# flanglet/kanzi-cpp

Hardware: AMD Instinct MI355X
Metric: encode+decode MB/s on the synthetic stand-in for silesia.tar (bit-exact) (higher is better)
Workload: dtype u8

## Files before the change

kanzi-cpp_amd/csrc/bwt_fwd.hip:

```cpp
#include "common.hpp"
#include "stages.hpp"
#include "bwt_common.hpp"

#include <cstdlib>
#include <cstring>
#include <algorithm>
#include <cmath>
#include "prims.hpp"
#include <chrono>
#include <vector>

namespace knz {

constexpr u32 SM_TS = 1792;
constexpr u32 SM_WIN = 2048;
constexpr u32 SM_G = 256;
constexpr u32 MED_CAP = 8192;
constexpr u32 MED_LO_CAP = 2048;
constexpr u32 SUPER_CAP = 8192;
constexpr int GATHER_THREADS = 512;
constexpr u32 GATHER_ROWS = 16;
static_assert(MED_CAP <= GATHER_ROWS * GATHER_THREADS, "k_bwt_f_gather_desc judges a medium group from one batch of loads");
constexpr u32 LARGE_OS_MIN = 1000000;
constexpr u32 NO_BIT = 0x7FFFFFFFu;
// ... 440 lines not shown
            if (tid + o < 64) sm = u < sm ? u : sm;
        }
        int pex = __shfl_up(pm, 1, 64);
        if (tid == 0) pex = -1;
        u32 sex = (u32)__shfl_down((int)sm, 1, 64);
        if (tid == 63) sex = NO_BIT;
        W.prevSet[tid] = pex;
        W.nextSet[tid] = sex;
        const bool zero = (tid < (int)(SM_TS / 32)) ? (w != 0xFFFFFFFFu) : (tid == (int)(SM_TS / 32) ? ((w & 1u) == 0) : false);
        const unsigned long long anyz = __ballot(zero);
        if (tid == 0) *sAny = anyz != 0 ? 1 : 0;
    }
    __syncthreads();
    return *sAny != 0;
}

__device__ __forceinline__ bool sm_group_of(const SmWindow& W, u32 i, u32& s, u32& e)
{
    const u32 w = i >> 5, bit = i & 31;
    const u32 lowmask = (bit == 31) ? 0xFFFFFFFFu : ((2u << bit) - 1u);
    const u32 word = W.bw[w];
    const u32 m = word & lowmask;
    int si = m ? (int)(w * 32 + 31 - __clz((int)m)) : W.prevSet[w];
    if (si < 0 || (u32)si >= SM_TS) return false;
    const u32 m2 = word & ~lowmask;
    const u32 ei = m2 ? (w * 32 + (u32)__ffs((int)m2) - 1) : W.nextSet[w];
    if (ei == NO_BIT) return false;
    const u32 len = ei - (u32)si;
    if (len < 2 || len > SM_G) return false;
    s = (u32)si; e = ei;
    return true;
}

__global__ __launch_bounds__(256) void k_bwt_f_r0_place_text(BwtView bv, FwdView v, const u32* __restrict__ winLastIncl, const u32* __restrict__ winFirstInclRev, u32 nWin,
                                                             uint2* __restrict__ largeNext, const u64* __restrict__ keys, int nsym, int pbits, uint2* __restrict__ runList,
                                                             const u32* __restrict__ gapTab)
{
    __shared__ SmWindow W;
    __shared__ int sBlk;
    __shared__ ClassAgg A;
    __shared__ u32 sSA[SM_WIN];
    __shared__ u64 sK[SM_WIN];
    __shared__ u32 sNew[64];
    __shared__ u32 sAfterLocal;
    constexpr int E = (int)(SM_WIN / 256);
    constexpr u32 TSW = SM_TS / 32;
    const int tid = (int)threadIdx.x;
    const u32 win = blockIdx.x;
    const u32 slot0 = win * SM_TS;
    if (tid == 0) sBlk = find_block(v.base, v.nBlocks, slot0 < v.total ? slot0 : v.total - 1);
    agg_init(A);
    if (tid < 64) {
        sNew[tid] = 0;
        const u32 w = v.gbits[(slot0 >> 5) + (u32)tid];
        W.bw[tid] = w;
        int pm = w ? (tid * 32 + 31 - __clz((int)w)) : -1;
        u32 sm = w ? (u32)(tid * 32 + __ffs((int)w) - 1) : NO_BIT;
        for (int o = 1; o < 64; o <<= 1) {
            const int t = __shfl_up(pm, (unsigned)o, 64);
            if (tid >= o) pm = t > pm ? t : pm;
            const u32 u = (u32)__shfl_down((int)sm, (unsigned)o, 64);
            if (tid + o < 64) sm = u < sm ? u : sm;
        }
        int pex = __shfl_up(pm, 1u, 64);
        if (tid == 0) pex = -1;
        u32 sex = (u32)__shfl_down((int)sm, 1u, 64);
        if (tid == 63) sex = NO_BIT;
        W.prevSet[tid] = pex;
        W.nextSet[tid] = sex;
    } else if (tid < 128) {
        const int k = tid - 64;
        const u32 w = (k < (int)(2 * TSW - 64)) ? v.gbits[(slot0 >> 5) + 64u + (u32)k] : 0u;
        const unsigned long long any = __ballot(w != 0);
        const int first = any ? __ffsll((long long)any) - 1 : 0;
        if (k == first) sAfterLocal = any ? SM_WIN + (u32)k * 32u + (u32)__ffs((int)w) - 1u : NO_BIT;
    }
    __syncthreads();
    const u32 before = win ? winLastIncl[win - 1] : 0u;
    u32 after = (sAfterLocal != NO_BIT) ? slot0 + sAfterLocal : ((win + 2 < nWin) ? winFirstInclRev[nWin - 3 - win] : v.total);
    if (after > v.total) after = v.total;
    const u64 pmask = (1ull << pbits) - 1ull;
    u32 gp[E], gs[E], ge[E];
    u64 kk[E];
    bool inView[E], mine[E];
    int blkOf[E];
#pragma unroll
    for (int k = 0; k < E; k++) {
        const u32 i = (u32)tid + 256u * (u32)k;
        const u32 a = slot0 + i;
        inView[k] = a < v.total;
        mine[k] = false; gp[k] = 0; kk[k] = 0; gs[k] = 0; ge[k] = 0; blkOf[k] = 0;
        if (!inView[k]) continue;
        int blk = sBlk;
        while (a >= v.base[blk + 1]) blk++;
        blkOf[k] = blk;
        kk[k] = keys[a];
        gp[k] = v.base[blk] + (u32)(kk[k] & pmask);
        mine[k] = sm_group_of(W, i, gs[k], ge[k]);
        if (mine[k]) {
            const u32 bb = v.base[blk], n = v.base[blk + 1] - bb;
            const u32 q = gp[k] - bb + (u32)nsym;
            const u8* t = bv.src[blk];
            const u64 x = text8(t, q, n);
            sSA[i] = gp[k];
            sK[i] = (__builtin_bswap64(x) & ~0xFFull) | (u64)(i - gs[k]);
        }
    }
    __syncthreads();
    u32 surv = 0;
    int hKind[E];
    u32 hLocal[E], hSize[E];
#pragma unroll
    for (int k = 0; k < E; k++) {
        const u32 i = (u32)tid + 256u * (u32)k;
        const u32 a = slot0 + i;
        hKind[k] = -1; hLocal[k] = 0; hSize[k] = 0;
        if (!inView[k]) continue;
        if (mine[k]) {
            const u64 ki = sK[i], lo = ki & ~0xFFull;
            u32 less = 0, rank = 0;
            for (u32 j = gs[k]; j < ge[k]; j++) {
                const u64 kj = sK[j];
                rank += (kj < ki) ? 1u : 0u;
                less += (kj < lo) ? 1u : 0u;
            }
            const u32 eqBefore = rank - less;
            const u32 headIdx = gs[k] + less;
            v.SA[slot0 + headIdx + eqBefore] = gp[k];
            lab_set(v, gp[k], v.base[blkOf[k]], slot0 + headIdx, slot0 + headIdx);
            if (less != 0 && eqBefore == 0) atomicOr(&sNew[headIdx >> 5], 1u << (headIdx & 31));
            if (eqBefore != 0) surv = 1;
            continue;
        }
        if (i >= SM_TS) continue;
        const u32 w = i >> 5, bit = i & 31;
        const u32 lowmask = (bit == 31) ? 0xFFFFFFFFu : ((2u << bit) - 1u);
        const u32 word = W.bw[w];
// ... 1784 lines not shown
        __syncthreads();
#pragma unroll
        for (u32 q = 0; q < RUN_ROWS / 4; q++) {
            const u32 row = wave + 4 * q;
            if (row >= nRows) break;
            const u32 Rend = rowMax[q] < c0 + RUN_CH - 1 ? rowMax[q] : c0 + RUN_CH - 1;
            for (u32 R = c0; R <= Rend; R++) {
                const bool alive = Lr[q] >= R;
                const unsigned long long m = __ballot(alive);
                const u32 j = segBase + colBase[R - c0] + cnt[row][R - c0] + (u32)__popcll(m & __lanemask_lt());
                if (alive && j < M) {
                    keys[j] = kb[q] | ((above ? hiAll - (u64)R : (u64)R) << kbits);
                    vals[j] = e[q] - R;
                    Rout[j] = R;
                }
            }
        }
        __syncthreads();
    }
}

__global__ __launch_bounds__(256) void k_bwt_f_run_flags(const u64* __restrict__ keys, u32 M, unsigned long long* __restrict__ bits64)
{
    const u32 j = blockIdx.x * 256 + threadIdx.x;
    const u64 k = (j < M) ? keys[j] : 0ull;
    u32 klo = (u32)__shfl_up((int)(u32)k, 1u, 64), khi = (u32)__shfl_up((int)(u32)(k >> 32), 1u, 64);
    u64 kp = ((u64)khi << 32) | klo;
    if ((threadIdx.x & 63) == 0 && j > 0 && j < M) kp = keys[j - 1];
    const bool f = (j >= M) || (j == 0) || (k != kp);
    const unsigned long long m = __ballot(f);
    if ((threadIdx.x & 63) == 0) bits64[j >> 6] = m;
}

__global__ __launch_bounds__(256) void k_bwt_f_run_place(FwdView v, const uint2* __restrict__ desc, const u32* __restrict__ loff, u32 M, int kbits, const u64* __restrict__ keys,
                                                         const u32* __restrict__ vals, const u32* __restrict__ bits, const u32* __restrict__ winLastIncl,
                                                         const u32* __restrict__ winFirstInclRev, u32 nWin, uint2* __restrict__ largeNext, const u32* __restrict__ memberR,
                                                         u32* __restrict__ ovr, u32* __restrict__ rtbits, const u32* __restrict__ lbase, int allLabels)
{
    __shared__ SmWindow W;
    __shared__ ClassAgg A;
    const int tid = (int)threadIdx.x;
    const u32 jb = blockIdx.x * 256u;
    const u32 win = jb / SM_WIN, j0 = win * SM_WIN;
    agg_init(A);
    if (tid < 64) {
        const u32 w = bits[(j0 >> 5) + (u32)tid];
        W.bw[tid] = w;
        int pm = w ? (tid * 32 + 31 - __clz((int)w)) : -1;
        u32 sm = w ? (u32)(tid * 32 + __ffs((int)w) - 1) : NO_BIT;
        for (int o = 1; o < 64; o <<= 1) {
            const int t = __shfl_up(pm, (unsigned)o, 64);
            if (tid >= o) pm = t > pm ? t : pm;
            const u32 u = (u32)__shfl_down((int)sm, (unsigned)o, 64);
            if (tid + o < 64) sm = u < sm ? u : sm;
        }
        int pex = __shfl_up(pm, 1u, 64);
        if (tid == 0) pex = -1;
        u32 sex = (u32)__shfl_down((int)sm, 1u, 64);
        if (tid == 63) sex = NO_BIT;
        W.prevSet[tid] = pex;
        W.nextSet[tid] = sex;
    }
    __syncthreads();
    const u32 j = jb + (u32)tid;
    u32 surv = 0, mySlot = 0, hLocal = 0, hSize = 0;
    int hKind = -1;
    bool setBit = false;
    if (j < M) {
        const u32 i = j - j0;
        const u32 w = i >> 5, bit = i & 31;
        const u32 lowmask = (bit == 31) ? 0xFFFFFFFFu : ((2u << bit) - 1u);
        const u32 word = W.bw[w];
        const u32 m = word & lowmask;
        const int si = m ? (int)(w * 32 + 31 - (u32)__clz((int)m)) : W.prevSet[w];
        const u32 nh = (si >= 0) ? j0 + (u32)si : (win ? winLastIncl[win - 1] : 0u);
        const u32 di = (u32)(keys[j] >> kbits);
        const u32 gs = desc[di].x, off = loff[di];
        const u32 gp = vals[j];
        mySlot = gs + (j - off);
        v.SA[mySlot] = gp;
        if (nh != off || allLabels) lab_set(v, gp, lbase[di], gs + (nh - off), gs);
        ovr[mySlot] = memberR[j];
        if (nh == j) {
            const u32 m2 = word & ~lowmask;
            const u32 ei = m2 ? (w * 32 + (u32)__ffs((int)m2) - 1) : W.nextSet[w];
            u32 nxt = (ei != NO_BIT) ? j0 + ei : ((win + 1 < nWin) ? winFirstInclRev[nWin - 2 - win] : M);
            if (nxt > M) nxt = M;
            setBit = (j != off);
            hSize = nxt - j;
            hKind = agg_note(A, hSize, false, surv, hLocal);
        }
    }
    if (__ballot(surv != 0) != 0 && (tid & 63) == 0) v.counters[CNT_SMALL_LEFT] = 1;
    __syncthreads();
    if (tid == 0) agg_reserve(A, v);
    __syncthreads();
    if (hKind >= 0) agg_write(A, v, hKind, hLocal, mySlot, hSize, largeNext, (uint2*)nullptr);
    const int lane = tid & 63;
    const bool live = j < M;
    const u32 s0 = (u32)__shfl((int)mySlot, 0, 64);
    const bool inLine = live && (mySlot == s0 + (u32)lane);
    const unsigned long long hm = __ballot(setBit && inLine), rm = __ballot(inLine);
    if (live && !inLine) {
        if (setBit) atomicOr(&v.gnew[mySlot >> 5], 1u << (mySlot & 31));
        atomicOr(&rtbits[mySlot >> 5], 1u << (mySlot & 31));
    }
    if (lane == 0) {
        const u32 w0 = s0 >> 5, sh = s0 & 31;
        for (int which = 0; which < 2; which++) {
            const unsigned long long mask = which ? rm : hm;
            u32* dst = which ? rtbits : v.gnew;
            if (mask == 0) continue;
            const u32 p0 = (u32)(mask << sh);
            const u32 p1 = sh ? (u32)(mask >> (32 - sh)) : (u32)(mask >> 32);
            const u32 p2 = sh ? (u32)(mask >> (64 - sh)) : 0u;
            if (p0) atomicOr(&dst[w0], p0);
            if (p1) atomicOr(&dst[w0 + 1], p1);
            if (p2) atomicOr(&dst[w0 + 2], p2);
        }
// ... 48 lines not shown
        d[0] = (u8)((logNbChunks << 2) | (pIndexSize - 1));
        u32 idx = 1;
        for (int k = 0; k < chunks; k++) {
            const u32 prim = lab_cur(fv, bb + (u32)k * step, bb) - bb;
            for (int sh = (int)(pIndexSize - 1) * 8; sh >= 0; sh -= 8) d[idx++] = (u8)(prim >> sh);
        }
        newLen[b] = hdr + n;
    }
}

__global__ __launch_bounds__(256) void k_bwt_f_med_flags(const uint2* __restrict__ stage, u32 nSlots, u32* __restrict__ flags)
{
    const u32 i = blockIdx.x * 256 + threadIdx.x;
    if (i >= nSlots) return;
    const u32 n = stage[i].y;
    flags[i] = (n != 0 && n <= MED_LO_CAP) ? 1u : 0u;
    flags[nSlots + i] = (n > MED_LO_CAP) ? 1u : 0u;
}

__global__ __launch_bounds__(256) void k_bwt_f_med_compact(uint2* __restrict__ stage, u32 nSlots, const u32* __restrict__ prefix, uint2* __restrict__ medNext,
                                                           u32 at, u32* __restrict__ idxLo, u32 atLo, u32* __restrict__ idxHi, u32 atHi, u32* __restrict__ nLoOut)
{
    const u32 i = blockIdx.x * 256 + threadIdx.x;
    if (i >= nSlots) return;
    const u32 nLo = prefix[nSlots];
    if (i == 0) *nLoOut = nLo;
    const uint2 d = stage[i];
    if (d.y == 0) return;
    const u32 pLo = prefix[i], pHi = prefix[nSlots + i] - nLo, g = at + pLo + pHi;
    medNext[g] = d; stage[i] = make_uint2(0u, 0u);
    if (d.y <= MED_LO_CAP) idxLo[atLo + pLo] = g; else idxHi[atHi + pHi] = g;
}

struct FwdTuning { int nsym; int noRunRound; int runFallback; int stats; int link; int plainLabels; int noPack; int noUnsplitSkip; int noGroupSleep; int noMediumFuse; int runSort; int chainList; int runInSort; };
static FwdTuning& fwd_tuning()
{
    static FwdTuning t = [] {
        FwdTuning x; x.nsym = 0; x.noRunRound = 0; x.runFallback = 0; x.stats = 0; x.link = 1; x.plainLabels = 0; x.noPack = 0; x.noUnsplitSkip = 0; x.noGroupSleep = 0; x.noMediumFuse = 0; x.runSort = 0; x.chainList = 0; x.runInSort = 0;
        if (getenv("KNZ_BWT_PLAIN_LABELS")) x.plainLabels = 1;
        if (getenv("KNZ_BWT_NO_PACK")) x.noPack = 1;
        if (getenv("KNZ_BWT_NO_UNSPLIT_SKIP")) x.noUnsplitSkip = 1;
        if (getenv("KNZ_BWT_NO_GROUP_SLEEP")) x.noGroupSleep = 1;
        if (getenv("KNZ_BWT_NO_MEDIUM_FUSE")) x.noMediumFuse = 1;
        if (const char* e = getenv("KNZ_BWT_RUN_SORT")) x.runSort = atoi(e);
        if (const char* e = getenv("KNZ_BWT_CHAIN_LIST")) x.chainList = atoi(e);
        if (const char* e = getenv("KNZ_BWT_RUN_IN_SORT")) x.runInSort = atoi(e);
        if (const char* e = getenv("KNZ_BWT_LINK")) x.link = atoi(e);
        if (getenv("KNZ_BWT_STATS")) x.stats = 1;
        if (const char* e = getenv("KNZ_BWT_NSYM")) x.nsym = atoi(e);
        if (getenv("KNZ_BWT_NO_RUN_ROUND")) x.noRunRound = 1;
        if (getenv("KNZ_BWT_RUN_FALLBACK")) x.runFallback = 1;
        return x;
    }();
    return t;
}
int bwt_forward_tune(const char* key, int value)
{
    FwdTuning& t = fwd_tuning();
    if (!strcmp(key, "rs_onesweep")) { prims::rs_onesweep_knob().store(value); return 0; }
    if (!strcmp(key, "bwt_nsym")) t.nsym = value;
    else if (!strcmp(key, "bwt_no_run_round")) t.noRunRound = value;
    else if (!strcmp(key, "bwt_run_fallback")) t.runFallback = value;
    else if (!strcmp(key, "bwt_stats")) t.stats = value;
    else if (!strcmp(key, "bwt_link")) t.link = value;
    else if (!strcmp(key, "bwt_plain_labels")) t.plainLabels = value;
    else if (!strcmp(key, "bwt_no_pack")) t.noPack = value;
    else if (!strcmp(key, "bwt_no_unsplit_skip")) t.noUnsplitSkip = value;
    else if (!strcmp(key, "bwt_no_group_sleep")) t.noGroupSleep = value;
    else if (!strcmp(key, "bwt_no_medium_fuse")) t.noMediumFuse = value;
    else if (!strcmp(key, "bwt_run_sort")) t.runSort = value;
    else if (!strcmp(key, "bwt_chain_list")) t.chainList = value;
    else if (!strcmp(key, "bwt_run_in_sort")) t.runInSort = value;
    else return -1;
    return 0;
}

struct FwdScratch {
    u64* keysA; u64* keysB;
    u32* valsA; u32* valsB;
    u32* SA; u32* ISA; u32* K; u64* ISA2;
    u32* t0; u32* t1; u32* t2; u32* t3;
    u32* gbits; u32* gnew; u32* rtbits; u32* ovr; size_t gbitsWords;
    uint2* med[2]; uint2* medStage; uint2* medVerdict[2]; u32* medFlags; u32* medPrefix; u32* medIdxLo; u32* medIdxHi; size_t medSlots; uint2* descInfo; uint2* large[2]; uint2* runList; uint4* superList; u32* ebits;
    u32* loff; u32* lbase;
    u32* survTile;
    u32* linkedTile;
    u32* base;
    u32* counters;
    u32* seg2;
    void* scanTmp;
    void* rsMem;
    u32* byteHist;
    u32* classTab; u32* rbits; u32* rcount; u32* rprefix;
    u32* runPos; u32* runE; u32* runL; u32* sE; u32* rcnt; u32* moff;
    u64* runKeysA; u64* runKeysB; u64* sKey;
    u32* runTileStart; u32* runColTab;
    u32* gapMembers; u32* gapFirst; u32* gapStart; u32* cbase;
    size_t maxRuns;
};

static size_t fwd_align(size_t x) { return (x + 255) & ~(size_t)255; }

static size_t fwd_carve(u8* p, int nBlocks, size_t total, FwdScratch* w, u32 VS)
{
    u8* q = p;
// ... 67 lines not shown
        if (mode == OFF && h >= retryH) mode = UNTRIED;
        if (mode == UNTRIED && survMembers >= total / 8) { mode = TRIAL; trials++; return true; }
        if (mode == ON && survMembers >= total / 64) { mode = APPLIED; return true; }
        return false;
    }
};

struct FwdSort {
    hipStream_t s; const XfStage& st; u32* hp;
    const FwdTuning tune = fwd_tuning();
    BwtView bv; FwdView v; FwdScratch w; size_t maxTotal;
    prims::RsWs rs1;
    u32 total, medSlots, nTiles; int nsym, pbits, kbits;
    bool groupSleep = false;
    u32 h = 1; int cur = 0;
    u64 *keysFree, *keysFree2;
    bool medFuse = false;
    bool runDirect = false;
    bool gaps = false;
    u32 gapClasses = 0, keptOut = 0, scanRuns = 0, scanLongest = 0;
    u32 nMedLo = 0;
    u32 nRun, runElems, surv, nMed, nLarge, largeElems, survMembers;
    LinkPlan link; LinkTrial linkTr; std::chrono::steady_clock::time_point statT;
    int fetch(u32 first, u32 n) { return hipMemcpyAsync(hp + first, w.counters + first, 4 * (size_t)n, hipMemcpyDeviceToHost, s) == hipSuccess && hipStreamSynchronize(s) == hipSuccess ? 0 : -1; }
    void merge_bits() { hipLaunchKernelGGL(k_bwt_f_merge_bits, GRID1(total / 32 + 2), w.gbits, w.gnew, total / 32 + 2); }
    void enable_run_tiebits() { if (!v.rtbits) { hipMemsetAsync(w.rtbits, 0, 4 * w.gbitsWords, s); v.ovr = w.ovr; v.rtbits = w.rtbits; } }
    void compact_medium(uint2* dst, u32 at = 0, u32 atLo = 0)
    {
        KScope ks_("k_bwt_f_med_compact");
        hipLaunchKernelGGL(k_bwt_f_med_flags, GRID1(medSlots), w.medStage, medSlots, w.medFlags);
        prims::launch_scan<prims::SCAN_SUM_EXCL>(s, w.medFlags, w.medPrefix, 2 * (size_t)medSlots, nullptr, w.scanTmp, w.counters + CNT_MED);
        hipLaunchKernelGGL(k_bwt_f_med_compact, GRID1(medSlots), w.medStage, medSlots, w.medPrefix, dst, at, w.medIdxLo, atLo, w.medIdxHi, at - atLo, w.counters + CNT_MED_LO);
    }
    void bounds(u32 n, bool last, const u32* bits = nullptr, u32 len = 0, u32 wordsPerWin = 0)
    {
        if (bits) { KScope ks_("k_bwt_f_r0_winsum"); hipLaunchKernelGGL(k_bwt_f_r0_winsum, GRID1(n), bits, len, n, w.t0, w.t2, wordsPerWin); }
        if (last) { KScope ks_("k_bwt_f_scan_max"); prims::launch_scan<prims::SCAN_MAX_INCL>(s, w.t0, w.t1, n, nullptr, w.scanTmp); }
        KScope ks_("k_bwt_f_scan_min"); prims::launch_scan<prims::SCAN_MIN_INCL>(s, w.t2, w.t3, n, nullptr, w.scanTmp);
    }
    template <class KEY, bool HAS_VAL> int sort_one_segment(u32 n, KEY* ka, KEY* kb, u32* va, u32* vb, int loBit, int hiBit, bool oneRead = true)
    {
        hipLaunchKernelGGL(prims::k_rs_one_segment, dim3(1), dim3(64), 0, s, w.seg2, n);
        prims::rs_launch_layout(s, rs1);
        return prims::rs_sort<KEY, HAS_VAL>(s, rs1, ka, kb, va, vb, (size_t)n, loBit, hiBit, oneRead);
    }
    int setup(void* scratch, size_t scratchBytes, BwtSuffixArrays* sa)
    {
        bv.src = st.src; bv.dst = st.dst; bv.len = st.len; bv.cap = st.cap; bv.VS = st.maxLen; bv.nBlocks = st.nBlocks;
        maxTotal = (size_t)st.nBlocks * bv.VS;
        if (fwd_carve(reinterpret_cast<u8*>(scratch), st.nBlocks, maxTotal, &w, bv.VS) > scratchBytes) return -2;
        { KScope ks_("k_bwt_f_bases"); hipLaunchKernelGGL(k_bwt_bases, dim3(1), dim3(64), 0, s, bv, w.base, st.ok, w.counters + CNT_LONGEST_BLOCK, sa ? 1 : 0); }
        hipMemsetAsync(st.newLen, 0, sizeof(u32) * st.nBlocks, s);
        { KScope ks_("k_bwt_f_r0_hist");
          hipMemsetAsync(w.byteHist, 0, 1024ull * st.nBlocks, s);
          hipLaunchKernelGGL(k_bwt_f_bytehist, dim3(64, (unsigned)st.nBlocks), dim3(256), 0, s, bv, w.base, w.byteHist);
          hipLaunchKernelGGL(k_bwt_f_choose_nsym, dim3(1), dim3(256), 0, s, w.byteHist, st.nBlocks, w.counters + CNT_LONGEST_BLOCK, w.counters + CNT_NSYM); }
        if (hipMemcpyAsync(hp, w.base + st.nBlocks, 4, hipMemcpyDeviceToHost, s) != hipSuccess || fetch(CNT_LONGEST_BLOCK, 2)) return -1;
        total = hp[0];
        if (sa) { sa->SA = w.SA; sa->base = w.base; sa->total = total; }
        if (total == 0) return 0;
        v.base = w.base; v.nBlocks = st.nBlocks; v.total = total; v.SA = w.SA; v.ISA = w.ISA; v.K = w.K; v.ISA2 = (w.ISA2 != nullptr && !tune.plainLabels) ? w.ISA2 : (u64*)nullptr;
        v.round = 0; v.gbits = w.gbits; v.gnew = w.gnew; v.counters = w.counters; v.medStage = w.medStage; v.ovr = nullptr; v.rtbits = nullptr;
        v.verdictNow = nullptr; v.verdictWas = nullptr;
        medSlots = (u32)((size_t)total / 256 + 1); nTiles = (total + SM_TS - 1) / SM_TS;
        survMembers = total;
        hipMemsetAsync(w.medStage, 0, 8ull * w.medSlots, s);
// ... 57 lines not shown
        }
        hipLaunchKernelGGL(k_bwt_f_r0_fill, dim3(128, (unsigned)st.nBlocks), dim3(256), 0, s, kin, w.gapMembers, w.gapStart, w.gapFirst, nsym, pbits);
        keysFree = kout; keysFree2 = kin;
    }
    void round0_sort()
    {
        const prims::RsWs rs = prims::rs_carve(w.rsMem, maxTotal, st.nBlocks + 1, w.base, st.nBlocks);
        rs1 = prims::rs_carve(w.rsMem, maxTotal, st.nBlocks + 1, w.seg2, 1);
        { KScope ks_("k_bwt_f_r0_layout"); prims::rs_launch_layout(s, rs); }
        u64* kin = w.keysA; u64* kout = w.keysB;
        const bool oneRead = one_read();
        if (gaps) { round0_sort_gaps(rs); return; }
        if (oneRead) {
            KScope ks_("k_bwt_f_r0_sort");
            hipLaunchKernelGGL(k_bwt_f_r0_counts, dim3((unsigned)rs.L.nSeg), dim3(256), 0, s, bv, w.base, w.byteHist, nsym, rs.L, (const u32*)nullptr);
            hipLaunchKernelGGL(prims::k_rs_digit_bases, dim3((unsigned)rs.L.nSeg, (unsigned)nsym), dim3(256), 0, s, rs.L);
        }
        auto sortPass = [&](const auto& src, int pass) {
            if (oneRead) prims::rs_launch_pass_os<u64, false>(s, rs, src, nullptr, kout, nullptr, (size_t)bv.VS, pass);
            else prims::rs_launch_pass<u64, false>(s, rs, src, nullptr, kout, nullptr, (size_t)bv.VS);
        };
        for (int pass = 0; pass < nsym; pass++) {
            KScope ks_("k_bwt_f_r0_sort");
            if (pass == 0) { TextSrc src; src.src = bv.src; src.P = nsym; src.pbits = pbits; src.shift = pbits; sortPass(src, pass); }
            else { prims::DigitOfKey<u64> src; src.keys = kin; src.shift = pbits + 8 * pass; src.mask = 255u; sortPass(src, pass); }
            std::swap(kin, kout);
        }
        keysFree = kout; keysFree2 = kin;
    }
    int round0_place()
    {
        hipMemsetAsync(w.gbits, 0xFF, 4 * w.gbitsWords, s); hipMemsetAsync(w.gnew, 0, 4 * w.gbitsWords, s);
        hipMemsetAsync(w.counters, 0, 4 * CNT_ROUND_SLOTS, s);
        { KScope ks_("k_bwt_f_r0_flags"); hipLaunchKernelGGL(k_bwt_f_r0_flags, dim3((total + 256 * R0F_ROWS - 1) / (256 * R0F_ROWS)), dim3(256), 0, s, keysFree2, w.base, st.nBlocks, total, nsym, pbits,
                                                             reinterpret_cast<unsigned long long*>(w.gbits)); }
        bounds(nTiles, true, w.gbits, total, SM_TS / 32);
        kbits = bits_for((u64)bv.VS + 2, 1);
        const bool runRound = (2 * kbits + 1) < 64 && !tune.noRunRound;
        { KScope ks_("k_bwt_f_r0_place");
          hipLaunchKernelGGL(k_bwt_f_r0_place_text, dim3(nTiles), dim3(256), 0, s, bv, v, w.t1, w.t3, nTiles, w.large[cur], keysFree2, nsym, pbits, runRound ? w.runList : (uint2*)nullptr,
                             gaps ? w.classTab : (const u32*)nullptr);
          merge_bits(); }
        if (fetch(0, CNT_ROUND_SLOTS)) return -1;
        nRun = hp[CNT_RUN]; runElems = hp[CNT_RUN_MEMBERS];
        return 0;
    }
    int run_fallback()
    {
        { KScope ks_("k_bwt_f_run_fallback"); hipLaunchKernelGGL(k_bwt_f_run_fallback, GRID1(nRun), v, w.runList, nRun, w.med[cur], w.large[cur]); }
        nRun = 0; return fetch(0, CNT_ROUND_SLOTS);
    }
    int run_round()
    {
        if (nRun && ((u64)nRun > (1ull << (64 - (2 * kbits + 1))) || tune.runFallback) && run_fallback()) return -1;
        if (gaps) {
            if (nRun != gapClasses || runElems != keptOut) return -1;
            { KScope ks_("k_bwt_f_run_classes"); hipLaunchKernelGGL(k_bwt_f_run_classes, GRID1(nRun), bv, v, w.runList, nRun, w.classTab); }
            return run_round_sorted(scanRuns, scanLongest);
        }
        if (!nRun) return 0;
        const u32 nWin = (total + SM_WIN - 1) / SM_WIN;
        { KScope ks_("k_bwt_f_run_ends"); hipLaunchKernelGGL(k_bwt_f_run_ends, dim3(nWin), dim3(256), 0, s, bv, v, reinterpret_cast<u8*>(w.ebits)); }
        bounds(nWin, false, w.ebits, total, SM_WIN / 32);
        hipMemsetAsync(w.classTab, 0xFF, 1024ull * (size_t)st.nBlocks, s);
        { KScope ks_("k_bwt_f_run_classes"); hipLaunchKernelGGL(k_bwt_f_run_classes, GRID1(nRun), bv, v, w.runList, nRun, w.classTab); }
        { KScope ks_("k_bwt_f_run_len"); hipLaunchKernelGGL(k_bwt_f_run_len<false>, dim3(nWin), dim3(256), 0, s, bv, v, w.ebits, w.t3, nWin, w.K, w.classTab, (u32)nsym,
                                                            reinterpret_cast<unsigned long long*>(w.rbits), w.rcount, (u32*)nullptr, (u32*)nullptr); }
        const u32 nRW = nWin * (SM_WIN / 32);
        { KScope ks_("k_bwt_f_scan_sum"); prims::launch_scan<prims::SCAN_SUM_EXCL>(s, w.rcount, w.rprefix, nRW, nullptr, w.scanTmp, w.counters + CNT_RUNS); }
        { KScope ks_("k_bwt_f_run_compact"); hipLaunchKernelGGL(k_bwt_f_run_compact, GRID1(nRW), w.rbits, w.rprefix, nRW, w.runPos); }
        if (fetch(CNT_RUN_LONGEST, 3)) return -1;
        return run_round_sorted(hp[CNT_RUNS], hp[CNT_RUN_LONGEST]);
    }
    int run_round_sorted(const u32 nRuns, const u32 longest)
// ... 6 lines not shown
                                                              gaps ? w.runList : (const uint2*)nullptr, (u32)nsym); }
        const u64* rkSorted;
        { KScope ks_("k_bwt_f_sort_runs");
          rkSorted = sort_one_segment<u64, false>(nRuns, w.runKeysA, w.runKeysB, nullptr, nullptr, idxBits, idxBits + kbits + 1 + rbits) ? w.runKeysB : w.runKeysA; }
        { KScope ks_("k_bwt_f_run_sorted"); hipLaunchKernelGGL(k_bwt_f_run_sorted, GRID1(nRuns), rkSorted, nRuns, idxBits, w.runE, w.runL, (u32)nsym, w.sE, w.sKey, w.rcnt); }
        { KScope ks_("k_bwt_f_scan_sum"); prims::launch_scan<prims::SCAN_SUM_EXCL>(s, w.rcnt, w.moff, nRuns, nullptr, w.scanTmp); }
        u64* rk; u32* rv = w.valsA;
        runDirect = !tune.runSort && longest <= RUN_DIRECT_LMAX;
        if (runDirect) {
            KScope ks_("k_bwt_f_run_direct");
            u32* segStart = w.runPos; u32* tileIdx = w.runE;
            const u32 maxTiles = (u32)std::min<u64>((u64)nRuns, 2ull * nRun + nRuns / RUN_TILE + 1);
            hipLaunchKernelGGL(k_bwt_f_run_seg_marks, GRID1(nRuns), w.sKey, nRuns, kbits, segStart);
            prims::launch_scan<prims::SCAN_MAX_INCL>(s, segStart, segStart, nRuns, nullptr, w.scanTmp);
            hipLaunchKernelGGL(k_bwt_f_run_tile_marks, GRID1(nRuns), segStart, nRuns, tileIdx);
            prims::launch_scan<prims::SCAN_SUM_EXCL>(s, tileIdx, tileIdx, nRuns, nullptr, w.scanTmp, w.counters + CNT_RUN_TILES);
            hipLaunchKernelGGL(k_bwt_f_run_tile_starts, GRID1(nRuns), segStart, tileIdx, nRuns, w.runTileStart);
            if (nRuns > RUN_TILE) {
                hipLaunchKernelGGL(k_bwt_f_run_tile_counts, dim3(maxTiles), dim3(256), 0, s, w.runTileStart, segStart, w.rcnt, nRuns, w.counters + CNT_RUN_TILES, (u32)nsym, w.runColTab);
                hipLaunchKernelGGL(k_bwt_f_run_tile_scan, dim3(maxTiles), dim3(256), 0, s, w.runTileStart, segStart, w.sKey, nRuns, w.counters + CNT_RUN_TILES, (u32)nsym, kbits, w.runColTab);
            }
            rk = keysFree;
            hipLaunchKernelGGL(k_bwt_f_run_emit, dim3(maxTiles), dim3(256), 0, s, w.runTileStart, segStart, w.rcnt, w.moff, w.sKey, w.sE, nRuns, runElems, w.counters + CNT_RUN_TILES,
                               w.runColTab, (u32)nsym, kbits, hbits, rk, rv, w.valsB);
        } else {
            { KScope ks_("k_bwt_f_run_members"); hipLaunchKernelGGL(k_bwt_f_run_members, dim3((runElems + 2047) / 2048), dim3(256), 0, s, w.moff, nRuns, runElems, w.sKey, kbits, hbits,
                                                                    (u32)nsym, keysFree); }
            KScope ks_("k_bwt_f_sort_members");
            const int r = sort_one_segment<u64, false>(runElems, keysFree, keysFree2, nullptr, nullptr, 32, 32 + hbits + rbits);
            rk = r ? keysFree : keysFree2;
            hipLaunchKernelGGL(k_bwt_f_run_expand, GRID1(runElems), r ? keysFree2 : keysFree, runElems, w.sKey, w.sE, kbits, hbits, rk, rv, w.valsB);
        }
        u32* mbits = w.ebits; const u32 nWinM = (runElems + SM_WIN - 1) / SM_WIN;
        { KScope ks_("k_bwt_f_large_flags"); hipLaunchKernelGGL(k_bwt_f_run_flags, dim3(nWinM * (SM_WIN / 256)), dim3(256), 0, s, rk, runElems, reinterpret_cast<unsigned long long*>(mbits)); }
        bounds(nWinM, true, mbits, runElems, SM_WIN / 32);
        { KScope ks_("k_bwt_f_large_place");
          hipMemsetAsync(w.rtbits, 0, 4 * w.gbitsWords, s);
          hipLaunchKernelGGL(k_bwt_f_run_place, dim3((runElems + 255) / 256), dim3(256), 0, s, v, w.runList, w.loff, runElems, hbits + kbits, rk, rv, mbits, w.t1, w.t3, nWinM, w.large[cur],
                             w.valsB, w.ovr, w.rtbits, w.lbase, gaps ? 1 : 0);
          v.ovr = w.ovr; v.rtbits = w.rtbits; }
        { KScope ks_("k_bwt_f_merge_bits"); merge_bits(); }
        return 0;
    }
    int probe()
    {
        u32* probeCand = w.medFlags;
        compact_medium(w.med[cur]);
        { KScope ks_("k_bwt_f_probe"); hipLaunchKernelGGL(k_bwt_f_probe_scan, dim3(256), dim3(256), 0, s, v, w.med[cur], (u32)nsym, v.rtbits, probeCand); }
        if (fetch(0, CNT_ROUND_SLOTS)) return -1;
        surv = hp[CNT_SMALL_LEFT]; nMed = hp[CNT_MED]; nMedLo = hp[CNT_MED_LO]; nLarge = hp[CNT_LARGE]; largeElems = hp[CNT_LARGE_MEMBERS];
        if (const u32 nCand = hp[CNT_PROBE_CAND]) {
            enable_run_tiebits();
            hipMemsetAsync(w.counters, 0, 4 * CNT_PROBE_SLOTS, s);
            { KScope ks_("k_bwt_f_probe");
              hipLaunchKernelGGL(k_bwt_f_probe, dim3(std::min<u32>(nCand, 4096)), dim3(512), 0, s, bv, v, w.med[cur], probeCand, nCand, (u32)nsym, w.med[cur ^ 1], w.large[cur], w.ovr, w.rtbits);
              merge_bits(); }
            compact_medium(w.med[cur], nMed, nMedLo);
            if (fetch(0, CNT_MED_LO + 1)) return -1;
            surv |= hp[CNT_SMALL_LEFT]; nMed += hp[CNT_MED]; nMedLo += hp[CNT_MED_LO];
        }
        if (tune.stats) fprintf(stderr, "after round 0 (nsym %d, total %u): run groups %u (%u members); small left %u, medium %u, large %u (%u members); run members placed directly %u, sorted %u, kept out of the round-0 sort %u\n",
                                nsym, total, nRun, runElems, surv, nMed, nLarge, largeElems, (nRun && runDirect) ? runElems : 0u, (nRun && !runDirect) ? runElems : 0u, gaps ? keptOut : 0u);
        statT = std::chrono::steady_clock::now();
        return 0;
    }
    void link_step()
    {
        KScope ks_("k_bwt_f_link");
        u32* posflag = w.ebits; u32* linked = w.rbits; u32* rev = w.rcount; u32* sufRev = w.rprefix;
        const bool trial = link.mode == LinkPlan::TRIAL; linkTr.n = 0;
        if (trial) { linkTr.blk[linkTr.n++] = 0; if (st.nBlocks >= 5) linkTr.blk[linkTr.n++] = st.nBlocks / 2; if (st.nBlocks >= 3) linkTr.blk[linkTr.n++] = st.nBlocks - 1; }
        const u32 nW = total / 32 + 1;
        hipMemsetAsync(posflag, 0, 4 * (size_t)nW, s);
// ... 121 lines not shown
```

Measured before the change: 7537.

## Fuse group-boundary flag computation into round-0 and run place kernels

The separate flag kernels and window-boundary scans that ran before the round-0 and run-round place kernels are dropped by default. Each place kernel now computes its own group-start flags from the sorted keys with wave ballots. It finds group bounds that cross a window edge through a wave-parallel search over neighbouring keys. This removes several kernel launches and a full pass over the keys, at the cost of extra global key reads and possibly long boundary searches inside the place kernels.

```diff
diff --git a/kanzi-cpp_amd/csrc/bwt_fwd.hip b/kanzi-cpp_amd/csrc/bwt_fwd.hip
--- a/kanzi-cpp_amd/csrc/bwt_fwd.hip
+++ b/kanzi-cpp_amd/csrc/bwt_fwd.hip
@@ -496,6 +496,66 @@
     return true;
 }
 
+template <class PRED>
+__device__ __forceinline__ u32 wave_first_true(u32 lo, u32 hi, PRED pred)
+{
+    const u32 lane = threadIdx.x & 63u;
+    for (int step = 0; step < 6 && lo < hi; step++) {
+        const u32 stride = (hi - lo + 63u) / 64u;
+        const u64 q = (u64)lo + (u64)(lane + 1u) * stride - 1ull;
+        const u32 p = q < (u64)hi ? (u32)q : hi - 1u;
+        const unsigned long long m = __ballot(pred(p));
+        if (m == 0) return hi;
+        const u32 f = (u32)__ffsll((long long)m) - 1u;
+        hi = (u32)__shfl((int)p, (int)f, 64);
+        lo += f * stride;
+    }
+    return hi;
+}
+template <class PRED>
+__device__ __forceinline__ u32 wave_first_true_up(u32 lo, u32 hi, PRED pred)
+{
+    const u32 mid = (hi - lo > 64u) ? lo + 64u : hi;
+    const u32 r = wave_first_true(lo, mid, pred);
+    return (r < mid || mid == hi) ? r : wave_first_true(mid, hi, pred);
+}
+template <class PRED>
+__device__ __forceinline__ u32 wave_first_true_down(u32 lo, u32 hi, PRED pred)
+{
+    const u32 mid = (hi - lo > 64u) ? hi - 64u : lo;
+    const u32 r = wave_first_true(mid, hi, pred);
+    return (r > mid || mid == lo) ? r : wave_first_true(lo, mid, pred);
+}
+
+__device__ __forceinline__ bool r0_short(u64 k, u64 pmask, int P, u32 n) { return (u32)(k & pmask) + (u32)P > n; }
+__device__ __forceinline__ bool r0_starts(u32 a, u32 bb, u32 n, u64 k, u64 kp, int P, int pbits)
+{
+    const u64 pm = (1ull << pbits) - 1ull;
+    return (a == bb) || ((k >> pbits) != (kp >> pbits)) || r0_short(k, pm, P, n) || r0_short(kp, pm, P, n);
+}
+
+__device__ __forceinline__ u32 r0_start_before(const u64* __restrict__ keys, u32 slot0, u32 bb, u32 n, int P, int pbits)
+{
+    const u32 lane = threadIdx.x & 63u;
+    const u64 S = keys[slot0] >> pbits, pm = (1ull << pbits) - 1ull;
+    const u32 lo = wave_first_true_down(bb, slot0, [&](u32 i) { return (keys[i] >> pbits) >= S; });
+    const u32 t = lo + lane;
+    const bool sh = (int)lane < P - 1 && t < slot0 && r0_short(keys[t], pm, P, n);
+    const unsigned long long m = __ballot(sh);
+    return m ? lo + 64u - (u32)__clzll((long long)m) : lo;
+}
+__device__ __forceinline__ u32 r0_start_after(const u64* __restrict__ keys, u32 last, u32 be, u32 n, int P, int pbits)
+{
+    const u32 lane = threadIdx.x & 63u;
+    const u64 S = keys[last] >> pbits, pm = (1ull << pbits) - 1ull;
+    const u32 hi = wave_first_true_up(last + 1u, be, [&](u32 i) { return (keys[i] >> pbits) != S; });
+    const u32 t = hi - 1u - lane;
+    const bool sh = (int)lane < P - 1 && lane < hi - 1u - last && r0_short(keys[t], pm, P, n);
+    const unsigned long long m = __ballot(sh);
+    return m ? hi - 64u + (u32)__clzll((long long)m) : hi;
+}
+
+template <bool FLAGS_PASS>
 __global__ __launch_bounds__(256) void k_bwt_f_r0_place_text(BwtView bv, FwdView v, const u32* __restrict__ winLastIncl, const u32* __restrict__ winFirstInclRev, u32 nWin,
                                                              uint2* __restrict__ largeNext, const u64* __restrict__ keys, int nsym, int pbits, uint2* __restrict__ runList,
                                                              const u32* __restrict__ gapTab)
@@ -503,21 +563,90 @@
     __shared__ SmWindow W;
     __shared__ int sBlk;
     __shared__ ClassAgg A;
-    __shared__ u32 sSA[SM_WIN];
     __shared__ u64 sK[SM_WIN];
     __shared__ u32 sNew[64];
     __shared__ u32 sAfterLocal;
+    __shared__ u32 sBeforeSlot;
     constexpr int E = (int)(SM_WIN / 256);
     constexpr u32 TSW = SM_TS / 32;
     const int tid = (int)threadIdx.x;
     const u32 win = blockIdx.x;
     const u32 slot0 = win * SM_TS;
+    const u64 pmask = (1ull << pbits) - 1ull;
+    u32 gp[E], gs[E], ge[E];
+    u64 kk[E];
+    bool inView[E], mine[E];
+    int blkOf[E];
     if (tid == 0) sBlk = find_block(v.base, v.nBlocks, slot0 < v.total ? slot0 : v.total - 1);
     agg_init(A);
+    if (tid < 64) sNew[tid] = 0;
+    if constexpr (FLAGS_PASS) {
+        if (tid < 64) {
+            W.bw[tid] = v.gbits[(slot0 >> 5) + (u32)tid];
+        } else if (tid < 128) {
+            const int k = tid - 64;
+            const u32 w = (k < (int)(2 * TSW - 64)) ? v.gbits[(slot0 >> 5) + 64u + (u32)k] : 0u;
+            const unsigned long long any = __ballot(w != 0);
+            const int first = any ? __ffsll((long long)any) - 1 : 0;
+            if (k == first) sAfterLocal = any ? SM_WIN + (u32)k * 32u + (u32)__ffs((int)w) - 1u : NO_BIT;
+        }
+    } else {
+        __syncthreads();
+        const int lane = tid & 63;
+        u64 kLeft = 0;
+        if (tid == 0 && slot0 > 0 && slot0 < v.total) kLeft = keys[slot0 - 1];
+#pragma unroll
+        for (int k = 0; k < E; k++) {
+            const u32 i = (u32)tid + 256u * (u32)k;
+            const u32 a = slot0 + i;
+            inView[k] = a < v.total;
+            kk[k] = keys[inView[k] ? a : v.total - 1u];
+        }
+#pragma unroll
+        for (int k = 0; k < E; k++) {
+            const u32 i = (u32)tid + 256u * (u32)k;
+            const u32 a = slot0 + i;
+            int blk = sBlk;
+            if (inView[k]) while (a >= v.base[blk + 1]) blk++;
+            blkOf[k] = blk;
+            if (!inView[k]) kk[k] = 0;
+            if (lane == 63) sK[i >> 6] = kk[k];
+        }
+        __syncthreads();
+#pragma unroll
+        for (int k = 0; k < E; k++) {
+            const u32 i = (u32)tid + 256u * (u32)k;
+            const u32 a = slot0 + i;
+            const u32 klo = (u32)__shfl_up((int)(u32)kk[k], 1u, 64), khi = (u32)__shfl_up((int)(u32)(kk[k] >> 32), 1u, 64);
+            u64 kp = ((u64)khi << 32) | klo;
+            if (lane == 0) kp = i ? sK[(i >> 6) - 1u] : kLeft;
+            bool f = true;
+            if (inView[k]) { const u32 bb = v.base[blkOf[k]]; f = r0_starts(a, bb, v.base[blkOf[k] + 1] - bb, kk[k], kp, nsym, pbits); }
+            const unsigned long long m = __ballot(f);
+            if (lane == 0) {
+                const u32 r = i >> 6;
+                W.bw[2u * r] = (u32)m; W.bw[2u * r + 1u] = (u32)(m >> 32);
+                if (2u * r < TSW) reinterpret_cast<unsigned long long*>(v.gbits)[(slot0 >> 6) + r] = m;
+            }
+        }
+        __syncthreads();
+        if (tid >= 64 && tid < 128) {
+            const u32 w = W.bw[lane];
+            const bool need = __ballot(lane >= (int)TSW && w != 0) == 0;
+            const u32 last = slot0 + SM_WIN - 1u;
+            u32 aft = v.total;
+            if (need && last + 1u < v.total) {
+                int blk = sBlk;
+                while (last >= v.base[blk + 1]) blk++;
+                const u32 bb = v.base[blk], be = v.base[blk + 1];
+                aft = last + 1u;
+                if (aft < be && !r0_starts(aft, bb, be - bb, keys[aft], keys[last], nsym, pbits)) aft = r0_start_after(keys, last, be, be - bb, nsym, pbits);
+            }
+            if (lane == 0) sAfterLocal = aft;
+        }
+    }
     if (tid < 64) {
-        sNew[tid] = 0;
-        const u32 w = v.gbits[(slot0 >> 5) + (u32)tid];
-        W.bw[tid] = w;
+        const u32 w = W.bw[tid];
         int pm = w ? (tid * 32 + 31 - __clz((int)w)) : -1;
         u32 sm = w ? (u32)(tid * 32 + __ffs((int)w) - 1) : NO_BIT;
         for (int o = 1; o < 64; o <<= 1) {
@@ -532,33 +661,35 @@
         if (tid == 63) sex = NO_BIT;
         W.prevSet[tid] = pex;
         W.nextSet[tid] = sex;
-    } else if (tid < 128) {
-        const int k = tid - 64;
-        const u32 w = (k < (int)(2 * TSW - 64)) ? v.gbits[(slot0 >> 5) + 64u + (u32)k] : 0u;
-        const unsigned long long any = __ballot(w != 0);
-        const int first = any ? __ffsll((long long)any) - 1 : 0;
-        if (k == first) sAfterLocal = any ? SM_WIN + (u32)k * 32u + (u32)__ffs((int)w) - 1u : NO_BIT;
-    }
-    __syncthreads();
-    const u32 before = win ? winLastIncl[win - 1] : 0u;
-    u32 after = (sAfterLocal != NO_BIT) ? slot0 + sAfterLocal : ((win + 2 < nWin) ? winFirstInclRev[nWin - 3 - win] : v.total);
+        if constexpr (!FLAGS_PASS) {
+            u32 bef = 0;
+            if ((W.bw[0] & 1u) == 0) { const u32 bb = v.base[sBlk]; bef = r0_start_before(keys, slot0, bb, v.base[sBlk + 1] - bb, nsym, pbits); }
+            if (tid == 0) sBeforeSlot = bef;
+        }
+    }
+    __syncthreads();
+    u32 before, after;
+    if constexpr (FLAGS_PASS) {
+        before = win ? winLastIncl[win - 1] : 0u;
+        after = (sAfterLocal != NO_BIT) ? slot0 + sAfterLocal : ((win + 2 < nWin) ? winFirstInclRev[nWin - 3 - win] : v.total);
+    } else {
+        before = sBeforeSlot; after = sAfterLocal;
+    }
     if (after > v.total) after = v.total;
-    const u64 pmask = (1ull << pbits) - 1ull;
-    u32 gp[E], gs[E], ge[E];
-    u64 kk[E];
-    bool inView[E], mine[E];
-    int blkOf[E];
 #pragma unroll
     for (int k = 0; k < E; k++) {
         const u32 i = (u32)tid + 256u * (u32)k;
         const u32 a = slot0 + i;
-        inView[k] = a < v.total;
-        mine[k] = false; gp[k] = 0; kk[k] = 0; gs[k] = 0; ge[k] = 0; blkOf[k] = 0;
+        if constexpr (FLAGS_PASS) { inView[k] = a < v.total; kk[k] = 0; blkOf[k] = 0; }
+        mine[k] = false; gp[k] = 0; gs[k] = 0; ge[k] = 0;
         if (!inView[k]) continue;
-        int blk = sBlk;
-        while (a >= v.base[blk + 1]) blk++;
-        blkOf[k] = blk;
-        kk[k] = keys[a];
+        int blk = blkOf[k];
+        if constexpr (FLAGS_PASS) {
+            blk = sBlk;
+            while (a >= v.base[blk + 1]) blk++;
+            blkOf[k] = blk;
+            kk[k] = keys[a];
+        }
         gp[k] = v.base[blk] + (u32)(kk[k] & pmask);
         mine[k] = sm_group_of(W, i, gs[k], ge[k]);
         if (mine[k]) {
@@ -566,7 +697,6 @@
             const u32 q = gp[k] - bb + (u32)nsym;
             const u8* t = bv.src[blk];
             const u64 x = text8(t, q, n);
-            sSA[i] = gp[k];
             sK[i] = (__builtin_bswap64(x) & ~0xFFull) | (u64)(i - gs[k]);
         }
     }
@@ -2417,59 +2547,104 @@
     if ((threadIdx.x & 63) == 0) bits64[j >> 6] = m;
 }
 
+template <bool FLAGS_PASS>
 __global__ __launch_bounds__(256) void k_bwt_f_run_place(FwdView v, const uint2* __restrict__ desc, const u32* __restrict__ loff, u32 M, int kbits, const u64* __restrict__ keys,
                                                          const u32* __restrict__ vals, const u32* __restrict__ bits, const u32* __restrict__ winLastIncl,
                                                          const u32* __restrict__ winFirstInclRev, u32 nWin, uint2* __restrict__ largeNext, const u32* __restrict__ memberR,
                                                          u32* __restrict__ ovr, u32* __restrict__ rtbits, const u32* __restrict__ lbase, int allLabels)
 {
-    __shared__ SmWindow W;
     __shared__ ClassAgg A;
     const int tid = (int)threadIdx.x;
     const u32 jb = blockIdx.x * 256u;
-    const u32 win = jb / SM_WIN, j0 = win * SM_WIN;
+    const u32 j = jb + (u32)tid;
     agg_init(A);
-    if (tid < 64) {
-        const u32 w = bits[(j0 >> 5) + (u32)tid];
-        W.bw[tid] = w;
-        int pm = w ? (tid * 32 + 31 - __clz((int)w)) : -1;
-        u32 sm = w ? (u32)(tid * 32 + __ffs((int)w) - 1) : NO_BIT;
-        for (int o = 1; o < 64; o <<= 1) {
-            const int t = __shfl_up(pm, (unsigned)o, 64);
-            if (tid >= o) pm = t > pm ? t : pm;
-            const u32 u = (u32)__shfl_down((int)sm, (unsigned)o, 64);
-            if (tid + o < 64) sm = u < sm ? u : sm;
-        }
-        int pex = __shfl_up(pm, 1u, 64);
-        if (tid == 0) pex = -1;
-        u32 sex = (u32)__shfl_down((int)sm, 1u, 64);
-        if (tid == 63) sex = NO_BIT;
-        W.prevSet[tid] = pex;
-        W.nextSet[tid] = sex;
-    }
-    __syncthreads();
-    const u32 j = jb + (u32)tid;
+    u32 nh = 0, nxt = 0;
+    const u64 key = (j < M) ? keys[j] : 0ull;
+    const u32 gp = (j < M) ? vals[j] : 0u, mR = (j < M) ? memberR[j] : 0u;
+    const u32 di = (u32)(key >> kbits);
+    u32 gs = 0, off = 0, lb = 0;
+    if (j < M) { gs = desc[di].x; off = loff[di]; lb = lbase[di]; }
+    if constexpr (FLAGS_PASS) {
+        __shared__ SmWindow W;
+        const u32 win = jb / SM_WIN, j0 = win * SM_WIN;
+        if (tid < 64) {
+            const u32 w = bits[(j0 >> 5) + (u32)tid];
+            W.bw[tid] = w;
+            int pm = w ? (tid * 32 + 31 - __clz((int)w)) : -1;
+            u32 sm = w ? (u32)(tid * 32 + __ffs((int)w) - 1) : NO_BIT;
+            for (int o = 1; o < 64; o <<= 1) {
+                const int t = __shfl_up(pm, (unsigned)o, 64);
+                if (tid >= o) pm = t > pm ? t : pm;
+                const u32 u = (u32)__shfl_down((int)sm, (unsigned)o, 64);
+                if (tid + o < 64) sm = u < sm ? u : sm;
+            }
+            int pex = __shfl_up(pm, 1u, 64);
+            if (tid == 0) pex = -1;
+            u32 sex = (u32)__shfl_down((int)sm, 1u, 64);
+            if (tid == 63) sex = NO_BIT;
+            W.prevSet[tid] = pex;
+            W.nextSet[tid] = sex;
+        }
+        __syncthreads();
+        if (j < M) {
+            const u32 i = j - j0;
+            const u32 w = i >> 5, bit = i & 31;
+            const u32 lowmask = (bit == 31) ? 0xFFFFFFFFu : ((2u << bit) - 1u);
+            const u32 word = W.bw[w];
+            const u32 m = word & lowmask;
+            const int si = m ? (int)(w * 32 + 31 - (u32)__clz((int)m)) : W.prevSet[w];
+            nh = (si >= 0) ? j0 + (u32)si : (win ? winLastIncl[win - 1] : 0u);
+            if (nh == j) {
+                const u32 m2 = word & ~lowmask;
+                const u32 ei = m2 ? (w * 32 + (u32)__ffs((int)m2) - 1) : W.nextSet[w];
+                nxt = (ei != NO_BIT) ? j0 + ei : ((win + 1 < nWin) ? winFirstInclRev[nWin - 2 - win] : M);
+            }
+        }
+    } else {
+        __shared__ unsigned long long sTie[4];
+        __shared__ u32 sOpen, sBeforeJ, sAfterJ;
+        const int lane = tid & 63, wv = tid >> 6;
+        const u32 klo = (u32)__shfl_up((int)(u32)key, 1u, 64), khi = (u32)__shfl_up((int)(u32)(key >> 32), 1u, 64);
+        u64 kp = ((u64)khi << 32) | klo;
+        if (lane == 0 && j > 0 && j < M) kp = keys[j - 1];
+        const bool f = (j >= M) || (j == 0) || (key != kp);
+        const unsigned long long mine = __ballot(f);
+        if (lane == 0) sTie[wv] = mine;
+        if (tid == 255) sOpen = (j + 1u < M && keys[j + 1u] == key) ? 1u : 0u;
+        __syncthreads();
+        if (wv == 0) {
+            u32 bef = jb;
+            if ((sTie[0] & 1ull) == 0) { const u64 K = keys[jb]; bef = wave_first_true_down(0u, jb, [&](u32 i) { return keys[i] == K; }); }
+            if (lane == 0) sBeforeJ = bef;
+        } else if (wv == 1) {
+            const u32 e = jb + 256u;
+            u32 aft = e < M ? e : M;
+            if (sOpen != 0 && (sTie[0] | sTie[1] | sTie[2] | sTie[3]) != 0) { const u64 K = keys[e - 1u]; aft = wave_first_true_up(e, M, [&](u32 i) { return keys[i] != K; }); }
+            if (lane == 0) sAfterJ = aft;
+        }
+        __syncthreads();
+        if (j < M) {
+            const unsigned long long upto = (lane == 63) ? ~0ull : ((2ull << lane) - 1ull);
+            unsigned long long m = mine & upto;
+            int w = wv;
+            while (m == 0 && w > 0) m = sTie[--w];
+            nh = m ? jb + (u32)w * 64u + 63u - (u32)__clzll((long long)m) : sBeforeJ;
+            if (f) {
+                m = mine & ~upto; w = wv;
+                while (m == 0 && w < 3) m = sTie[++w];
+                nxt = m ? jb + (u32)w * 64u + (u32)__ffsll((long long)m) - 1u : sAfterJ;
+            }
+        }
+    }
     u32 surv = 0, mySlot = 0, hLocal = 0, hSize = 0;
     int hKind = -1;
     bool setBit = false;
     if (j < M) {
-        const u32 i = j - j0;
-        const u32 w = i >> 5, bit = i & 31;
-        const u32 lowmask = (bit == 31) ? 0xFFFFFFFFu : ((2u << bit) - 1u);
-        const u32 word = W.bw[w];
-        const u32 m = word & lowmask;
-        const int si = m ? (int)(w * 32 + 31 - (u32)__clz((int)m)) : W.prevSet[w];
-        const u32 nh = (si >= 0) ? j0 + (u32)si : (win ? winLastIncl[win - 1] : 0u);
-        const u32 di = (u32)(keys[j] >> kbits);
-        const u32 gs = desc[di].x, off = loff[di];
-        const u32 gp = vals[j];
         mySlot = gs + (j - off);
         v.SA[mySlot] = gp;
-        if (nh != off || allLabels) lab_set(v, gp, lbase[di], gs + (nh - off), gs);
-        ovr[mySlot] = memberR[j];
+        if (nh != off || allLabels) lab_set(v, gp, lb, gs + (nh - off), gs);
+        ovr[mySlot] = mR;
         if (nh == j) {
-            const u32 m2 = word & ~lowmask;
-            const u32 ei = m2 ? (w * 32 + (u32)__ffs((int)m2) - 1) : W.nextSet[w];
-            u32 nxt = (ei != NO_BIT) ? j0 + ei : ((win + 1 < nWin) ? winFirstInclRev[nWin - 2 - win] : M);
             if (nxt > M) nxt = M;
             setBit = (j != off);
             hSize = nxt - j;
@@ -2584,11 +2759,11 @@
     if (d.y <= MED_LO_CAP) idxLo[atLo + pLo] = g; else idxHi[atHi + pHi] = g;
 }
 
-struct FwdTuning { int nsym; int noRunRound; int runFallback; int stats; int link; int plainLabels; int noPack; int noUnsplitSkip; int noGroupSleep; int noMediumFuse; int runSort; int chainList; int runInSort; };
+struct FwdTuning { int nsym; int noRunRound; int runFallback; int stats; int link; int plainLabels; int noPack; int noUnsplitSkip; int noGroupSleep; int noMediumFuse; int runSort; int chainList; int runInSort; int placeFlagsPass; };
 static FwdTuning& fwd_tuning()
 {
     static FwdTuning t = [] {
-        FwdTuning x; x.nsym = 0; x.noRunRound = 0; x.runFallback = 0; x.stats = 0; x.link = 1; x.plainLabels = 0; x.noPack = 0; x.noUnsplitSkip = 0; x.noGroupSleep = 0; x.noMediumFuse = 0; x.runSort = 0; x.chainList = 0; x.runInSort = 0;
+        FwdTuning x; x.nsym = 0; x.noRunRound = 0; x.runFallback = 0; x.stats = 0; x.link = 1; x.plainLabels = 0; x.noPack = 0; x.noUnsplitSkip = 0; x.noGroupSleep = 0; x.noMediumFuse = 0; x.runSort = 0; x.chainList = 0; x.runInSort = 0; x.placeFlagsPass = 0;
         if (getenv("KNZ_BWT_PLAIN_LABELS")) x.plainLabels = 1;
         if (getenv("KNZ_BWT_NO_PACK")) x.noPack = 1;
         if (getenv("KNZ_BWT_NO_UNSPLIT_SKIP")) x.noUnsplitSkip = 1;
@@ -2597,6 +2772,7 @@
         if (const char* e = getenv("KNZ_BWT_RUN_SORT")) x.runSort = atoi(e);
         if (const char* e = getenv("KNZ_BWT_CHAIN_LIST")) x.chainList = atoi(e);
         if (const char* e = getenv("KNZ_BWT_RUN_IN_SORT")) x.runInSort = atoi(e);
+        if (const char* e = getenv("KNZ_BWT_PLACE_FLAGS_PASS")) x.placeFlagsPass = atoi(e);
         if (const char* e = getenv("KNZ_BWT_LINK")) x.link = atoi(e);
         if (getenv("KNZ_BWT_STATS")) x.stats = 1;
         if (const char* e = getenv("KNZ_BWT_NSYM")) x.nsym = atoi(e);
@@ -2623,6 +2799,7 @@
     else if (!strcmp(key, "bwt_run_sort")) t.runSort = value;
     else if (!strcmp(key, "bwt_chain_list")) t.chainList = value;
     else if (!strcmp(key, "bwt_run_in_sort")) t.runInSort = value;
+    else if (!strcmp(key, "bwt_place_flags_pass")) t.placeFlagsPass = value;
     else return -1;
     return 0;
 }
@@ -2756,6 +2933,15 @@
         prims::launch_scan<prims::SCAN_SUM_EXCL>(s, w.medFlags, w.medPrefix, 2 * (size_t)medSlots, nullptr, w.scanTmp, w.counters + CNT_MED);
         hipLaunchKernelGGL(k_bwt_f_med_compact, GRID1(medSlots), w.medStage, medSlots, w.medPrefix, dst, at, w.medIdxLo, atLo, w.medIdxHi, at - atLo, w.counters + CNT_MED_LO);
     }
+    int bit_stats(const char* what, const u32* bitsDev, u32 n, bool flagsPass)
+    {
+        std::vector<u32> hb((size_t)n / 32 + 1);
+        if (hipMemcpyAsync(hb.data(), bitsDev, 4 * hb.size(), hipMemcpyDeviceToHost, s) != hipSuccess || hipStreamSynchronize(s) != hipSuccess) return -1;
+        u64 count = 0, sum = 0;
+        for (u32 a = 0; a < n; a++) if ((hb[a >> 5] >> (a & 31)) & 1u) { count++; sum += (u64)a + 1ull; }
+        fprintf(stderr, "%s: %llu set, checksum %llu (%s)\n", what, (unsigned long long)count, (unsigned long long)sum, flagsPass ? "flag pass" : "placing kernel");
+        return 0;
+    }
     void bounds(u32 n, bool last, const u32* bits = nullptr, u32 len = 0, u32 wordsPerWin = 0)
     {
         if (bits) { KScope ks_("k_bwt_f_r0_winsum"); hipLaunchKernelGGL(k_bwt_f_r0_winsum, GRID1(n), bits, len, n, w.t0, w.t2, wordsPerWin); }
@@ -2879,14 +3065,18 @@
     {
         hipMemsetAsync(w.gbits, 0xFF, 4 * w.gbitsWords, s); hipMemsetAsync(w.gnew, 0, 4 * w.gbitsWords, s);
         hipMemsetAsync(w.counters, 0, 4 * CNT_ROUND_SLOTS, s);
-        { KScope ks_("k_bwt_f_r0_flags"); hipLaunchKernelGGL(k_bwt_f_r0_flags, dim3((total + 256 * R0F_ROWS - 1) / (256 * R0F_ROWS)), dim3(256), 0, s, keysFree2, w.base, st.nBlocks, total, nsym, pbits,
-                                                             reinterpret_cast<unsigned long long*>(w.gbits)); }
-        bounds(nTiles, true, w.gbits, total, SM_TS / 32);
+        const bool flagsPass = tune.placeFlagsPass == 1 || tune.placeFlagsPass == 2;
+        if (flagsPass) {
+            { KScope ks_("k_bwt_f_r0_flags"); hipLaunchKernelGGL(k_bwt_f_r0_flags, dim3((total + 256 * R0F_ROWS - 1) / (256 * R0F_ROWS)), dim3(256), 0, s, keysFree2, w.base, st.nBlocks, total, nsym, pbits,
+                                                                 reinterpret_cast<unsigned long long*>(w.gbits)); }
+            bounds(nTiles, true, w.gbits, total, SM_TS / 32);
+        }
         kbits = bits_for((u64)bv.VS + 2, 1);
         const bool runRound = (2 * kbits + 1) < 64 && !tune.noRunRound;
         { KScope ks_("k_bwt_f_r0_place");
-          hipLaunchKernelGGL(k_bwt_f_r0_place_text, dim3(nTiles), dim3(256), 0, s, bv, v, w.t1, w.t3, nTiles, w.large[cur], keysFree2, nsym, pbits, runRound ? w.runList : (uint2*)nullptr,
-                             gaps ? w.classTab : (const u32*)nullptr);
+          hipLaunchKernelGGL(flagsPass ? k_bwt_f_r0_place_text<true> : k_bwt_f_r0_place_text<false>, dim3(nTiles), dim3(256), 0, s, bv, v, w.t1, w.t3, nTiles, w.large[cur], keysFree2, nsym, pbits,
+                             runRound ? w.runList : (uint2*)nullptr, gaps ? w.classTab : (const u32*)nullptr);
+          if (tune.stats && bit_stats("round 0 group starts", w.gbits, total, flagsPass)) return -1;
           merge_bits(); }
         if (fetch(0, CNT_ROUND_SLOTS)) return -1;
         nRun = hp[CNT_RUN]; runElems = hp[CNT_RUN_MEMBERS];
@@ -2959,13 +3149,17 @@
             hipLaunchKernelGGL(k_bwt_f_run_expand, GRID1(runElems), r ? keysFree2 : keysFree, runElems, w.sKey, w.sE, kbits, hbits, rk, rv, w.valsB);
         }
         u32* mbits = w.ebits; const u32 nWinM = (runElems + SM_WIN - 1) / SM_WIN;
-        { KScope ks_("k_bwt_f_large_flags"); hipLaunchKernelGGL(k_bwt_f_run_flags, dim3(nWinM * (SM_WIN / 256)), dim3(256), 0, s, rk, runElems, reinterpret_cast<unsigned long long*>(mbits)); }
-        bounds(nWinM, true, mbits, runElems, SM_WIN / 32);
+        const bool flagsPass = tune.placeFlagsPass == 1 || tune.placeFlagsPass == 3;
+        if (flagsPass) {
+            { KScope ks_("k_bwt_f_large_flags"); hipLaunchKernelGGL(k_bwt_f_run_flags, dim3(nWinM * (SM_WIN / 256)), dim3(256), 0, s, rk, runElems, reinterpret_cast<unsigned long long*>(mbits)); }
+            bounds(nWinM, true, mbits, runElems, SM_WIN / 32);
+        }
         { KScope ks_("k_bwt_f_large_place");
           hipMemsetAsync(w.rtbits, 0, 4 * w.gbitsWords, s);
-          hipLaunchKernelGGL(k_bwt_f_run_place, dim3((runElems + 255) / 256), dim3(256), 0, s, v, w.runList, w.loff, runElems, hbits + kbits, rk, rv, mbits, w.t1, w.t3, nWinM, w.large[cur],
-                             w.valsB, w.ovr, w.rtbits, w.lbase, gaps ? 1 : 0);
+          hipLaunchKernelGGL(flagsPass ? k_bwt_f_run_place<true> : k_bwt_f_run_place<false>, dim3((runElems + 255) / 256), dim3(256), 0, s, v, w.runList, w.loff, runElems, hbits + kbits, rk, rv, mbits,
+                             w.t1, w.t3, nWinM, w.large[cur], w.valsB, w.ovr, w.rtbits, w.lbase, gaps ? 1 : 0);
           v.ovr = w.ovr; v.rtbits = w.rtbits; }
+        if (tune.stats && bit_stats("run round tie starts", w.gnew, total, flagsPass)) return -1;
         { KScope ks_("k_bwt_f_merge_bits"); merge_bits(); }
         return 0;
     }
```

New measurement: 7524. No clear change (-0.2%).
